# nihalsid/single-view-3d-reconstruction

Hardware: AMD Instinct MI355X
Metric: query-points/sec fwd+bwd (128^3 grid, 50k pts) (higher is better)
Workload: dtype f32

## Files before the change

include/svr_hip.h:

```cpp
#ifndef SVR_HIP_H
#define SVR_HIP_H

#include <stdint.h>

#ifdef __cplusplus
extern "C" {
#endif

#define SVR_OK 0
#define SVR_E_BADARG (-1)
#define SVR_E_BADSHAPE (-2)
#define SVR_E_ALIGN (-3)
#define SVR_E_UNSUPPORTED (-4)
#define SVR_E_IO (-5)
#define SVR_E_NOTFOUND (-6)

#define SVR_MAX_LEVELS 6

int svr_version(void);
const char *svr_last_error(void);

typedef struct svr_pull_plan {
  const uint32_t *keys;
  const void *recs;
  const int32_t *heads;
  int64_t n_items;
} svr_pull_plan;

typedef struct svr_level {
  const float *vol;
  float *gvol;
  int32_t C, D, H, W;
  int32_t col;
  const int32_t *order;
  const int32_t *item_order;
  const svr_pull_plan *plan;
} svr_level;

typedef struct svr_gather_desc {
  int32_t n_levels;
  int32_t B, N;
  int32_t row_stride;
  int32_t align_corners;
  float displacement;
  const int32_t *order;
  svr_level level[SVR_MAX_LEVELS];
  int32_t flags;
} svr_gather_desc;

#define SVR_GATHER_WIDE_OFFSETS 1
#define SVR_GATHER_DETERMINISTIC 2

int64_t svr_sizeof_level(void);
int64_t svr_sizeof_gather_desc(void);

int svr_points_voxel_order(const float *points, int32_t *order, int32_t B, int32_t N, int32_t D, int32_t H,
                           int32_t W, int32_t align_corners, void *workspace, void *stream);
int64_t svr_points_morton_order_workspace(int32_t B, int32_t N);
int svr_points_morton_order(const float *points, int32_t *order, float *sorted_points ,
                            int32_t B, int32_t N, void *workspace, void *stream);

int64_t svr_gather_pull_plan_workspace(int32_t B, int32_t N);
int64_t svr_gather_pull_plan_workspace_cells(int32_t B, int32_t D, int32_t H, int32_t W);
int svr_gather_pull_plan(const float *points, int32_t B, int32_t N, int32_t D, int32_t H, int32_t W, int32_t C,
                         int32_t col, int32_t row_stride, int32_t align_corners, float displacement,
                         uint32_t *keys, void *recs, int32_t *heads, int32_t *items , int32_t *stats ,
                         void *workspace, void *stream);

int svr_gather_item_order(const float *points, int32_t B, int32_t N, int32_t D, int32_t H, int32_t W,
                          int32_t align_corners, float displacement, int32_t with_j ,
                          int32_t *items, void *workspace, void *stream);
int svr_gather_item_order_xblock(const float *points, int32_t B, int32_t N, int32_t D, int32_t H, int32_t W,
                                 int32_t align_corners, float displacement, int32_t block, int32_t *items,
                                 void *workspace, void *stream);
int svr_gather_project_bwd(const float *points, const float *dh, int64_t lddh, int32_t B, int32_t N, int32_t D, int32_t H,
                           int32_t W, int32_t align_corners, float displacement, const int32_t *items, float *dP,
                           void *stream);

int64_t svr_gather_project_plan_workspace(int32_t B, int32_t N);
int64_t svr_gather_project_slots(int32_t B, int32_t N, int32_t D, int32_t H, int32_t W);
int svr_gather_project_plan(const float *points, int32_t B, int32_t N, int32_t D, int32_t H, int32_t W, int32_t align_corners,
                            float displacement, int32_t *items, uint32_t *keys, int32_t *sidx, int32_t *first_slot,
                            void *workspace, void *stream);
int svr_gather_project_bwd2(const float *points, const float *dh, int64_t lddh, int32_t B, int32_t N, int32_t D, int32_t H,
                            int32_t W, int32_t align_corners, float displacement, const int32_t *items, const int32_t *sidx,
                            const int32_t *first_slot, float *partials, float *dP, void *stream);

int svr_gather_trilinear_fwd(const svr_gather_desc *d, const float *points ,
                             float *features, void *stream);
int32_t svr_gather_fc0_supported(const svr_gather_desc *d);
int64_t svr_gather_fc0_workspace(const svr_gather_desc *d, int32_t n_out);
int svr_gather_fc0_fwd(const svr_gather_desc *d, const float *points, const float *W, int64_t ldw, const float *bias, float *Y,
                       int64_t ldy, int32_t n_out, float *features, int64_t ldf, const int32_t *keep_cols, uint32_t keep_levels,
                       int32_t epilogue, void *workspace, void *stream);
int svr_gather_fc0_prepare(const svr_gather_desc *d, const float *W, int64_t ldw, int32_t n_out, float *features, int64_t ldf,
                           const int32_t *keep_cols, uint32_t keep_levels, void *workspace, void *stream);
int svr_gather_fc0_run(const svr_gather_desc *d, const float *points, const float *bias, float *Y, int64_t ldy, int32_t n_out,
                       float *features, int64_t ldf, const int32_t *keep_cols, uint32_t keep_levels, int32_t epilogue,
                       void *workspace, void *stream);
int svr_gather_fc0_bf16_prepare(const svr_gather_desc *d, const float *W, int64_t ldw, int32_t n_out, void *workspace,
                                void *stream);
int svr_gather_fc0_bf16_run(const svr_gather_desc *d, const float *points, const float *bias, uint16_t *Y, int64_t ldy,
                            int32_t n_out, int32_t epilogue, void *workspace, void *stream);
int svr_gather_trilinear_bwd(const svr_gather_desc *d, const float *points, const float *gfeatures,
                             float *gpoints, void *stream);
int svr_gather_corner_indices(const svr_gather_desc *d, int32_t level, const float *points,
                              int32_t *out, void *stream);

int svr_cast_f32_to_bf16(const float *in, uint16_t *out, int64_t n, void *stream);
int svr_gather_trilinear_fwd_bf16(const svr_gather_desc *d, const float *points, uint16_t *features, void *stream);
int svr_linear_fwd_bf16(const uint16_t *X, int64_t ldx, const uint16_t *W, int64_t ldw, const float *bias, uint16_t *Y,
                        int64_t ldy, int64_t M, int64_t N, int64_t K, int epilogue, void *stream);
int svr_fc_out_fwd_bf16(const uint16_t *H, int64_t ldh, const float *w, const float *b, float *logits,
                        const int32_t *row_map, int64_t M, int64_t K, void *stream);

#define SVR_EPI_NONE 0
#define SVR_EPI_BIAS 1
#define SVR_EPI_BIAS_RELU 2
#define SVR_EPI_MASK 3

int svr_linear_fwd(const float *X, int64_t ldx, const float *W, int64_t ldw, const float *bias,
                   float *Y, int64_t ldy, int64_t M, int64_t N, int64_t K, int epilogue,
                   const float *mask, int64_t ldmask, void *stream);
int svr_linear_bwd_data(const float *dY, int64_t lddy, const float *W, int64_t ldw, float *dX,
                        int64_t lddx, int64_t M, int64_t N, int64_t K, int epilogue,
                        const float *mask, int64_t ldmask, void *stream);
int64_t svr_linear_bwd_weight_workspace(int64_t M, int64_t N, int64_t K);
int svr_linear_bwd_weight(const float *dY, int64_t lddy, const float *X, int64_t ldx, float *dW,
                          int64_t lddw, float *db, int64_t M, int64_t N, int64_t K,
                          void *workspace, void *stream);

int64_t svr_linear_fwd_bf16x6_workspace(int64_t N, int64_t K);
int svr_linear_fwd_bf16x6(const float *X, int64_t ldx, const float *W, int64_t ldw, const float *bias,
                          float *Y, int64_t ldy, int64_t M, int64_t N, int64_t K, int epilogue,
// ... 366 lines not shown
```

single-view-3d-reconstruction_amd/_lib.py:

```python
import ctypes as C
import os

import numpy as np
import torch

_HERE = os.path.dirname(os.path.abspath(__file__))
LIB_PATH = os.path.join(_HERE, "lib", "libsvr_hip.so")

SVR_MAX_LEVELS = 6
EPI_NONE, EPI_BIAS, EPI_BIAS_RELU, EPI_MASK = 0, 1, 2, 3

P = C.c_void_p
I32, I64, F32 = C.c_int32, C.c_int64, C.c_float


class Conv2dDesc(C.Structure):
    _fields_ = [("src0", P), ("src1", P), ("B", I32), ("H", I32), ("W", I32), ("C0", I32), ("C1", I32), ("k", I32),
                ("stride", I32), ("act", I32), ("upsample", I32)]


class PullPlan(C.Structure):
    _fields_ = [("keys", P), ("recs", P), ("heads", P), ("n_items", I64)]


class Level(C.Structure):
    _fields_ = [("vol", P), ("gvol", P), ("C", I32), ("D", I32), ("H", I32), ("W", I32), ("col", I32), ("order", P),
                ("item_order", P), ("plan", C.POINTER(PullPlan))]


class GatherDesc(C.Structure):
    _fields_ = [("n_levels", I32), ("B", I32), ("N", I32), ("row_stride", I32), ("align_corners", I32),
                ("displacement", F32), ("order", P), ("level", Level * SVR_MAX_LEVELS), ("flags", I32)]


GATHER_WIDE_OFFSETS, GATHER_DETERMINISTIC = 1, 2
EVAL_SUMS_WORKSPACE_BYTES = 6144


SIGNATURES = {
    "svr_version": (C.c_int, []),
    "svr_last_error": (C.c_char_p, []),
    "svr_sizeof_level": (I64, []),
    "svr_sizeof_gather_desc": (I64, []),
    "svr_points_morton_order_workspace": (I64, [I32, I32]),
    "svr_points_morton_order": (C.c_int, [P, P, P, I32, I32, P, P]),
    "svr_points_voxel_order": (C.c_int, [P, P, I32, I32, I32, I32, I32, I32, P, P]),
    "svr_gather_item_order": (C.c_int, [P, I32, I32, I32, I32, I32, I32, F32, I32, P, P, P]),
    "svr_gather_item_order_xblock": (C.c_int, [P, I32, I32, I32, I32, I32, I32, F32, I32, P, P, P]),
    "svr_gather_project_bwd": (C.c_int, [P, P, I64, I32, I32, I32, I32, I32, I32, F32, P, P, P]),
    "svr_gather_project_plan_workspace": (C.c_int64, [I32, I32]),
    "svr_gather_project_slots": (C.c_int64, [I32, I32, I32, I32, I32]),
    "svr_gather_project_plan": (C.c_int, [P, I32, I32, I32, I32, I32, I32, F32, P, P, P, P, P, P]),
    "svr_gather_project_bwd2": (C.c_int, [P, P, I64, I32, I32, I32, I32, I32, I32, F32, P, P, P, P, P, P]),
    "svr_gather_pull_plan_workspace": (I64, [I32, I32]),
    "svr_gather_pull_plan_workspace_cells": (I64, [I32, I32, I32, I32]),
    "svr_gather_pull_plan": (C.c_int, [P, I32, I32, I32, I32, I32, I32, I32, I32, I32, F32, P, P, P, P, P, P, P]),
    "svr_gather_trilinear_fwd": (C.c_int, [C.POINTER(GatherDesc), P, P, P]),
    "svr_gather_fc0_supported": (C.c_int32, [C.POINTER(GatherDesc)]),
    "svr_gather_fc0_workspace": (C.c_int64, [C.POINTER(GatherDesc), I32]),
    "svr_gather_fc0_fwd": (C.c_int, [C.POINTER(GatherDesc), P, P, I64, P, P, I64, I32, P, I64, P, C.c_uint32, I32, P, P]),
    "svr_gather_fc0_prepare": (C.c_int, [C.POINTER(GatherDesc), P, I64, I32, P, I64, P, C.c_uint32, P, P]),
    "svr_gather_fc0_run": (C.c_int, [C.POINTER(GatherDesc), P, P, P, I64, I32, P, I64, P, C.c_uint32, I32, P, P]),
    "svr_gather_fc0_bf16_prepare": (C.c_int, [C.POINTER(GatherDesc), P, I64, I32, P, P]),
    "svr_gather_fc0_bf16_run": (C.c_int, [C.POINTER(GatherDesc), P, P, P, I64, I32, I32, P, P]),
    "svr_gather_trilinear_bwd": (C.c_int, [C.POINTER(GatherDesc), P, P, P, P]),
    "svr_gather_corner_indices": (C.c_int, [C.POINTER(GatherDesc), I32, P, P, P]),
    "svr_cast_f32_to_bf16": (C.c_int, [P, P, I64, P]),
    "svr_gather_trilinear_fwd_bf16": (C.c_int, [C.POINTER(GatherDesc), P, P, P]),
    "svr_linear_fwd_bf16": (C.c_int, [P, I64, P, I64, P, P, I64, I64, I64, I64, C.c_int, P]),
    "svr_fc_out_fwd_bf16": (C.c_int, [P, I64, P, P, P, P, I64, I64, P]),
    "svr_linear_fwd": (C.c_int, [P, I64, P, I64, P, P, I64, I64, I64, I64, C.c_int, P, I64, P]),
    "svr_linear_bwd_data": (C.c_int, [P, I64, P, I64, P, I64, I64, I64, I64, C.c_int, P, I64, P]),
    "svr_linear_bwd_weight_workspace": (I64, [I64, I64, I64]),
    "svr_linear_bwd_weight": (C.c_int, [P, I64, P, I64, P, I64, P, I64, I64, I64, P, P]),
    "svr_linear_fwd_bf16x6_workspace": (I64, [I64, I64]),
    "svr_linear_fwd_bf16x6": (C.c_int, [P, I64, P, I64, P, P, I64, I64, I64, I64, C.c_int, P, P]),
    "svr_linear_fwd_f16x3_workspace": (I64, [I64, I64]),
    "svr_linear_fwd_f16x3": (C.c_int, [P, I64, P, I64, P, P, I64, I64, I64, I64, C.c_int, P, P]),
    "svr_linear_bwd_data_bf16x3_workspace": (I64, [I64, I64]),
    "svr_linear_bwd_data_bf16x3": (C.c_int, [P, I64, P, I64, P, I64, I64, I64, I64, C.c_int, P, I64, P, P]),
    "svr_linear_bwd_weight_bf16x3_workspace": (I64, [I64, I64, I64]),
    "svr_linear_bwd_weight_bf16x3": (C.c_int, [P, I64, P, I64, P, I64, P, I64, I64, I64, P, P]),
    "svr_amax_f32": (C.c_int, [P, I64, I64, I64, P, P]),
    "svr_linear_bwd_data_f16x3_workspace": (I64, [I64, I64]),
    "svr_linear_bwd_data_f16x3": (C.c_int, [P, I64, P, I64, P, I64, I64, I64, I64, C.c_int, P, I64, P, P, P, P]),
    "svr_linear_bwd_weight_f16x3_workspace": (I64, [I64, I64, I64]),
    "svr_linear_bwd_weight_f16x3": (C.c_int, [P, I64, P, I64, P, I64, P, I64, I64, I64, P, P, P]),
    "svr_linear_variant": (C.c_int, [I32, I64, I64, I64, I64, I64, I64, I64, I32, I32, I32, I32, I32, I32, P, P, P, P, P, P]),
    "svr_fc_out_fwd": (C.c_int, [P, I64, P, P, P, P, I64, I64, P]),
    "svr_fc_out_bwd_workspace": (I64, [I64, I64]),
    "svr_fc_out_bwd": (C.c_int, [P, I64, P, P, P, P, I64, P, P, I64, I64, P, P, P]),
    "svr_bce_logits_sum_mean": (C.c_int, [P, P, P, P, I64, I64, F32, P, P]),
    "svr_bce_ordered_workspace": (I64, [I64]),
    "svr_bce_logits_sum_mean_ordered": (C.c_int, [P, P, P, P, I64, I64, F32, P, P]),
    "svr_conv3d_pack_weight": (C.c_int, [P, P, P, I32, I32, P]),
    "svr_conv3d_unpack_wgrad": (C.c_int, [P, P, I32, I32, P]),
    "svr_conv3d_k3": (C.c_int, [P, P, P, P, I32, I32, I32, I32, I32, I32, C.c_int, P, P]),
    "svr_conv3d_fwd_bf16x6_workspace": (I64, [I32, I32]),
    "svr_conv3d_k3_fwd_bf16x6": (C.c_int, [P, P, P, P, I32, I32, I32, I32, I32, I32, C.c_int, P, P]),
    "svr_conv3d_fwd_f16x3_workspace": (I64, [I32, I32]),
    "svr_conv3d_k3_fwd_f16x3": (C.c_int, [P, P, P, P, I32, I32, I32, I32, I32, I32, C.c_int, P, P]),
    "svr_conv3d_fwd_f16x3_stats_blocks": (I32, [I32, I32, I32, I32, I32, I32]),
    "svr_conv3d_k3_fwd_f16x3_stats": (C.c_int, [P, P, P, P, P, I32, I32, I32, I32, I32, I32, C.c_int, P, P]),
    "svr_conv3d_bwd_data_bf16x3_workspace": (I64, [I32, I32]),
    "svr_conv3d_k3_bwd_data_bf16x3": (C.c_int, [P, P, P, I32, I32, I32, I32, I32, I32, C.c_int, P, P, P]),
    "svr_conv3d_c1_fwd_stats_workspace": (I64, [I32, I32, I32, I32, I32]),
    "svr_conv3d_c1_fwd_stats": (C.c_int, [P, P, P, P, P, I32, I32, I32, I32, I32, C.c_int, P, P]),
    "svr_conv3d_k3_bwd_weight_workspace": (I64, [I32, I32, I32, I32, I32, I32]),
    "svr_conv3d_k3_bwd_weight": (C.c_int, [P, P, P, P, I32, I32, I32, I32, I32, I32, P, P]),
    "svr_conv3d_k3_bwd_weight_bf16x3_workspace": (I64, [I32, I32, I32, I32, I32, I32]),
    "svr_conv3d_k3_bwd_weight_bf16x3": (C.c_int, [P, P, P, P, I32, I32, I32, I32, I32, I32, P, P]),
    "svr_conv3d_k3_bwd_weight_bf16x3_param": (C.c_int, [P, P, P, P, I32, I32, I32, I32, I32, I32, P, P]),
    "svr_conv3d_bwd_data_f16x3_workspace": (I64, [I32, I32]),
    "svr_conv3d_k3_bwd_data_f16x3": (C.c_int, [P, P, P, I32, I32, I32, I32, I32, I32, C.c_int, P, P, P, P, P]),
    "svr_conv3d_k3_bwd_weight_f16x3": (C.c_int, [P, P, P, P, I32, I32, I32, I32, I32, I32, I32, P, P, P]),
    "svr_conv3d_k3_variant": (C.c_int, [I32, I32, I32, I32, I32, I32, I32, P, P, P, P, P]),
    "svr_bn_stats_workspace": (I64, [I64, I32]),
    "svr_bn_stats": (C.c_int, [P, P, I64, I32, P, P]),
# ... 167 lines not shown
```

single-view-3d-reconstruction_amd/csrc/gather.hip:

```cpp
#include "common.h"
#include "gather_common.h"
#include "reduce.h"

namespace {

struct LevelArgs {
  const float *vol;
  float *gvol;
  int C, D, H, W, col;
  const int32_t *order;
  const int32_t *items;
};

struct FusedArgs {
  LevelArgs L[SVR_MAX_LEVELS];
  unsigned block_start[SVR_MAX_LEVELS + 1];
  int n;
  int pad_start;
  int shared;
  int xcd;
};

template <int C, bool JMAJOR = false>
__device__ __forceinline__ void gather_fwd_body(const LevelArgs L, const float *__restrict__ points,
// ... 715 lines not shown
}

__global__ __launch_bounds__(128) void gather_bwd_serial_kernel(LevelArgs L, const float *__restrict__ points,
                                                                const float *__restrict__ gfeat, int N,
                                                                int row_stride, float disp, int ac) {
  const int b = blockIdx.x, c = threadIdx.x;
  if (c >= L.C) return;
  float *gb = L.gvol + (size_t)b * L.D * L.H * L.W * L.C + c;
  for (int j = 0; j < 7; ++j)
    for (int n = 0; n < N; ++n) {
      const int64_t pn = (int64_t)b * N + n;
      const Corner cr = sample_corner(points + pn * 3, j, disp, L.D, L.H, L.W, ac);
      const Weights w = corner_weights(cr);
      const float g = gfeat[pn * row_stride + L.col + j * L.C + c];
#pragma unroll
      for (int k = 0; k < 8; ++k) {
        const int z = w.z0 + (k >> 2), y = w.y0 + ((k >> 1) & 1), x = w.x0 + (k & 1);
        if (z >= 0 && z < L.D && y >= 0 && y < L.H && x >= 0 && x < L.W) {
          volatile float *q = gb + (((size_t)z * L.H + y) * L.W + x) * L.C;
          *q = *q + corner_w(w, k) * g;
        }
      }
    }
}

struct PullRec {
  float fx, fy, fz;
  int32_t goff;
};

__device__ __forceinline__ bool pull_cell(const float *pt, int j, float disp, int D, int H, int W, int ac, int b,
                                          uint32_t &key, float &fx, float &fy, float &fz) {
  const Corner c = sample_corner(pt, j, disp, D, H, W, ac);
  const int x0 = clamp_int(c.x0f), y0 = clamp_int(c.y0f), z0 = clamp_int(c.z0f);
  fx = c.ix - c.x0f;
  fy = c.iy - c.y0f;
  fz = c.iz - c.z0f;
  if (!(z0 >= -1 && z0 < D && y0 >= -1 && y0 < H && x0 >= -1 && x0 < W)) return false;
  key = (uint32_t)((((int64_t)b * (D + 1) + z0 + 1) * (H + 1) + y0 + 1) * (W + 1) + x0 + 1);
  return true;
}

__global__ __launch_bounds__(256) void pull_key_kernel(const float *__restrict__ points, uint32_t *__restrict__ keys,
                                                       int32_t *__restrict__ vals, int64_t total, int N, int D, int H,
                                                       int W, float disp, int ac, uint32_t sentinel, int kblk) {
  const int64_t i = (int64_t)blockIdx.x * 256 + threadIdx.x;
  if (i >= total) return;
  const int64_t pn = i / 7;
  const int j = (int)(i - pn * 7);
  uint32_t key;
  float fx, fy, fz;
  const float p3[3] = {points[pn * 3], points[pn * 3 + 1], points[pn * 3 + 2]};
  const bool ok = pull_cell(p3, j, disp, D, H, W, ac, (int)(pn / N), key, fx, fy, fz);
  if (ok && kblk > 0) {
    const uint32_t w1 = (uint32_t)W + 1u, K = (uint32_t)kblk, row = key / w1, x = key - row * w1;
    key = ((row * ((w1 + K - 1u) / K) + x / K) * 8u + (uint32_t)j) * K + x % K;
  }
  keys[i] = ok ? key : sentinel;
  vals[i] = (int32_t)i;
}

__global__ __launch_bounds__(256) void pull_record_kernel(const float *__restrict__ points,
                                                          const uint32_t *__restrict__ keys,
                                                          const int32_t *__restrict__ items, PullRec *__restrict__ recs,
                                                          int32_t *__restrict__ ends, int64_t total, int N, int D, int H,
                                                          int W, int C, int col, int row_stride, float disp, int ac,
                                                          uint32_t sentinel) {
  const int64_t idx = (int64_t)blockIdx.x * 256 + threadIdx.x;
  if (idx >= total) return;
  const uint32_t k = keys[idx];
  if (k == sentinel) return;
  const int32_t id = items[idx];
  const int32_t pn = id / 7;
  const int j = id - pn * 7;
  const float p3[3] = {points[(int64_t)pn * 3], points[(int64_t)pn * 3 + 1], points[(int64_t)pn * 3 + 2]};
  uint32_t key;
  PullRec r;
  pull_cell(p3, j, disp, D, H, W, ac, pn / N, key, r.fx, r.fy, r.fz);
  r.goff = pn * row_stride + col + j * C;
  recs[idx] = r;
  if (idx == total - 1 || keys[idx + 1] != k) ends[k + 1] = (int32_t)idx + 1;
}

template <int C, int XS, int BZ, int BY, int BXG>
__global__ __launch_bounds__(256) void gather_bwd_pull_kernel(float *__restrict__ gvol, const uint32_t *__restrict__ keys,
                                                              const PullRec *__restrict__ recs,
                                                              const int32_t *__restrict__ cs,
                                                              const float *__restrict__ gfeat, int n_items, int B, int D,
                                                              int H, int W) {
  constexpr int V = C / 4;
  static_assert(BZ * BY * BXG * V == 256, "brick must fill the workgroup");
  const int t = threadIdx.x;
  const int q4 = (t % V) * 4, si = t / V;
  const int nbx = (W + BXG * XS - 1) / (BXG * XS), nby = (H + BY - 1) / BY, nbz = (D + BZ - 1) / BZ;
  uint32_t bid = blockIdx.x;
  const int bx = bid % nbx; bid /= nbx;
  const int by = bid % nby; bid /= nby;
  const int bz = bid % nbz;
  const int b = bid / nbz;
  const int x0 = (bx * BXG + si % BXG) * XS, y = by * BY + (si / BXG) % BY, z = bz * BZ + si / (BXG * BY);
  if (x0 >= W || y >= H || z >= D) return;
  const int ncell = min(XS, W - x0) + 1;
  uint32_t kbase[4];
  int lo[4], hi[4];
#pragma unroll
  for (int w = 0; w < 4; ++w) {
    const int dz = w >> 1, dy = w & 1;
    kbase[w] = (uint32_t)((((int64_t)b * (D + 1) + z + dz) * (H + 1) + y + dy) * (W + 1) + x0);
    lo[w] = cs[kbase[w]];
    hi[w] = cs[kbase[w] + ncell];
  }
  float4 acc[XS];
#pragma unroll
  for (int i = 0; i < XS; ++i) acc[i] = make_float4(0.f, 0.f, 0.f, 0.f);
  const int last = n_items - 1;
  while (lo[0] < hi[0] || lo[1] < hi[1] || lo[2] < hi[2] || lo[3] < hi[3]) {
    uint32_t k[4];
    PullRec r[4];
#pragma unroll
    for (int w = 0; w < 4; ++w) {
      const int i = min(lo[w], last);
      k[w] = keys[i];
      r[w] = recs[i];
    }
    float4 g[4];
    bool v[4];
#pragma unroll
    for (int w = 0; w < 4; ++w) {
      v[w] = lo[w] < hi[w];
      g[w] = *reinterpret_cast<const float4 *>(gfeat + (v[w] ? r[w].goff : 0) + q4);
    }
#pragma unroll
    for (int w = 0; w < 4; ++w) {
      const int dz = w >> 1, dy = w & 1;
      if (v[w]) {
        const int o = (int)(k[w] - kbase[w]);
        const float wyz = (dy ? 1.f - r[w].fy : r[w].fy) * (dz ? 1.f - r[w].fz : r[w].fz);
        const float wa = r[w].fx * wyz, wb = (1.f - r[w].fx) * wyz;
#pragma unroll
        for (int i = 0; i < XS; ++i) {
          const float wt = (o == i) ? wa : ((o == i + 1) ? wb : 0.f);
          acc[i].x += wt * g[w].x; acc[i].y += wt * g[w].y; acc[i].z += wt * g[w].z; acc[i].w += wt * g[w].w;
        }
        ++lo[w];
      }
    }
  }
  float *out = gvol + ((((int64_t)b * D + z) * H + y) * W + x0) * C + q4;
#pragma unroll
  for (int i = 0; i < XS; ++i)
    if (x0 + i < W) *reinterpret_cast<float4 *>(out + (int64_t)i * C) = acc[i];
}

template <int XS>
__global__ __launch_bounds__(256) void gather_bwd_pull_c1_kernel(float *__restrict__ gvol, const uint32_t *__restrict__ keys,
                                                                 const PullRec *__restrict__ recs,
                                                                 const int32_t *__restrict__ cs,
                                                                 const float *__restrict__ gfeat, int n_items,
                                                                 int64_t strips, int D, int H, int W) {
  const int64_t t = (int64_t)blockIdx.x * 256 + threadIdx.x;
  if (t >= strips) return;
  const int nsx = (W + XS - 1) / XS;
  const int x0 = (int)(t % nsx) * XS;
  int64_t q = t / nsx;
  const int y = (int)(q % H); q /= H;
  const int z = (int)(q % D);
  const int64_t b = q / D;
  const int ncell = min(XS, W - x0) + 1;
  uint32_t kbase[4];
  int lo[4], hi[4];
#pragma unroll
  for (int w = 0; w < 4; ++w) {
    const int dz = w >> 1, dy = w & 1;
    kbase[w] = (uint32_t)(((b * (D + 1) + z + dz) * (H + 1) + y + dy) * (W + 1) + x0);
    lo[w] = cs[kbase[w]];
    hi[w] = cs[kbase[w] + ncell];
  }
  float acc[XS];
#pragma unroll
  for (int i = 0; i < XS; ++i) acc[i] = 0.f;
  const int last = n_items > 0 ? n_items - 1 : 0;
  while (lo[0] < hi[0] || lo[1] < hi[1] || lo[2] < hi[2] || lo[3] < hi[3]) {
    uint32_t k[4];
    PullRec r[4];
#pragma unroll
    for (int w = 0; w < 4; ++w) {
      const int i = min(lo[w], last);
      k[w] = keys[i];
      r[w] = recs[i];
    }
    float g[4];
    bool v[4];
#pragma unroll
    for (int w = 0; w < 4; ++w) {
      v[w] = lo[w] < hi[w];
      g[w] = gfeat[v[w] ? r[w].goff : 0];
    }
#pragma unroll
    for (int w = 0; w < 4; ++w) {
      const int dz = w >> 1, dy = w & 1;
      if (v[w]) {
        const int o = (int)(k[w] - kbase[w]);
        const float wyz = (dy ? 1.f - r[w].fy : r[w].fy) * (dz ? 1.f - r[w].fz : r[w].fz);
        const float wa = r[w].fx * wyz, wb = (1.f - r[w].fx) * wyz;
#pragma unroll
        for (int i = 0; i < XS; ++i) {
          const float wt = (o == i) ? wa : ((o == i + 1) ? wb : 0.f);
          acc[i] += wt * g[w];
        }
        ++lo[w];
      }
    }
  }
  float *out = gvol + ((b * D + z) * H + y) * (int64_t)W + x0;
#pragma unroll
  for (int i = 0; i < XS; ++i)
    if (x0 + i < W) out[i] = acc[i];
}

__host__ __device__ inline int pull_xs(int C) { return C == 16 ? 8 : 4; }

__global__ __launch_bounds__(256) void pull_stats_kernel(const int32_t *__restrict__ cs, int32_t *__restrict__ stats, int B, int D,
                                                         int H, int W, int XS) {
  const int nsx = (W + XS - 1) / XS;
  const int64_t total = (int64_t)B * (D + 1) * (H + 1) * nsx, i = (int64_t)blockIdx.x * 256 + threadIdx.x;
  int len = 0;
  if (i < total) {
    const int sx = (int)(i % nsx);
    const int64_t row = i / nsx;
    const int x0 = sx * XS, ncell = min(XS, W - x0) + 1;
// ... 50 lines not shown
                                        void *stream) {
  if (int rc = check_desc(d, false)) return rc;
  if ((int64_t)d->B * d->N == 0) return SVR_OK;
  SVR_CHECK(points && features, SVR_E_BADARG, "gather_fwd: null points/features");
  SVR_CHECK(((uintptr_t)features & 15) == 0, SVR_E_ALIGN, "gather_fwd: features not 16-byte aligned");
  hipStream_t s = (hipStream_t)stream;
  int64_t BN = (int64_t)d->B * d->N;
  if (BN == 0) return SVR_OK;
  FusedArgs A;
  A.n = 0;
  unsigned blocks = 0;
  bool shared = BN * (int64_t)d->row_stride < (1LL << 31) && !(d->flags & SVR_GATHER_WIDE_OFFSETS);
  for (int l = 0; l < d->n_levels; ++l)
    if ((int64_t)d->B * d->level[l].D * d->level[l].H * d->level[l].W * d->level[l].C >= (1LL << 31)) shared = false;
  A.shared = shared ? 1 : 0;
  for (int pass = 0; pass < 2; ++pass)
    for (int l = d->n_levels - 1; l >= 0; --l) {
      if ((d->level[l].C >= 4) != (pass == 0)) continue;
      LevelArgs L = level_args(d->level[l]);
      int V = L.C >= 4 ? L.C / 4 : 1;
      A.L[A.n] = L;
      A.block_start[A.n] = blocks;
      blocks += svr::xcd_grid((shared && L.C >= 16) ? svr::cdiv(BN * 7, 256) : svr::cdiv(BN * 7 * V, 256));
      ++A.n;
    }
  A.block_start[A.n] = blocks;
  static const int xcd_order = getenv("SVR_GATHER_XCD") ? 1 : 0;
  A.xcd = xcd_order;
  A.pad_start = 0;
  for (int l = 0; l < d->n_levels; ++l) {
    int end = d->level[l].col + 7 * d->level[l].C;
    if (end > A.pad_start) A.pad_start = end;
  }
  hipLaunchKernelGGL(gather_fwd_fused_kernel, dim3(blocks), dim3(256), 0, s, A, points, features, d->order, BN, d->N,
                     d->row_stride, d->displacement, d->align_corners);
  return svr::launch_status("gather_fwd");
}

extern "C" int svr_gather_trilinear_bwd(const svr_gather_desc *d, const float *points, const float *gfeatures,
                                        float *gpoints, void *stream) {
  if (int rc = check_desc(d, true)) return rc;
  if ((int64_t)d->B * d->N == 0) return SVR_OK;
  SVR_CHECK(points && gfeatures, SVR_E_BADARG, "gather_bwd: null points/gfeatures");
  hipStream_t s = (hipStream_t)stream;
  int64_t BN = (int64_t)d->B * d->N;
  if (BN == 0) return SVR_OK;
  if (gpoints) {
    hipError_t e = hipMemsetAsync(gpoints, 0, (size_t)BN * 3 * sizeof(float), s);
    SVR_CHECK(e == hipSuccess, (int)e, "gather_bwd: memset failed: %s", hipGetErrorString(e));
  }
  FusedArgs FA;
  FA.n = 0;
  unsigned fblocks = 0;
  for (int l = d->n_levels - 1; l >= 0; --l) {
    LevelArgs L = level_args(d->level[l]);
    bool gv = L.gvol != nullptr;
    if (!gv && !gpoints) continue;
    SVR_CHECK(L.vol != nullptr || !gpoints, SVR_E_BADARG, "gather_bwd: level %d needs vol for the point gradient", l);
    if (gpoints) {
      int V = L.C >= 4 ? L.C / 4 : 1;
      int64_t total = BN * 7 * V;
      unsigned grid = (unsigned)svr::cdiv(total, 256);
      DISPATCH_C(L.C, hipLaunchKernelGGL((gather_bwd_kernel<CC, false, true>), dim3(grid), dim3(256), 0, s, L, points,
                                         gfeatures, gpoints, total, d->N, d->row_stride, d->displacement,
                                         d->align_corners));
    }
    if (!gv) continue;
    if (d->level[l].plan && !(d->flags & SVR_GATHER_DETERMINISTIC)) {
      const svr_pull_plan *P = d->level[l].plan;
      SVR_CHECK(L.C == 1 || L.C == 16 || L.C == 32 || L.C == 64, SVR_E_UNSUPPORTED, "gather_bwd: level %d: pull plan with C=%d", l,
                L.C);
      SVR_CHECK(P->keys && P->recs && P->heads && P->n_items == 7 * BN, SVR_E_BADARG, "gather_bwd: level %d: bad pull plan", l);
      SVR_CHECK(P->n_items < (1LL << 31) && BN * (int64_t)d->row_stride < (1LL << 31), SVR_E_UNSUPPORTED,
                "gather_bwd: level %d: pull plan needs 32-bit item / gradient offsets", l);
      const int n = (int)P->n_items;
      const PullRec *recs = (const PullRec *)P->recs;
#define SVR_PULL(CC, XS, BZ, BY, BXG)                                                                                     \
  {                                                                                                                       \
    const int64_t blocks = (int64_t)d->B * svr::cdiv(L.D, BZ) * svr::cdiv(L.H, BY) * svr::cdiv(L.W, BXG * XS);            \
    SVR_CHECK(blocks < (1LL << 31), SVR_E_UNSUPPORTED, "gather_bwd: level %d: %ld pull workgroups", l, (long)blocks);     \
    hipLaunchKernelGGL((gather_bwd_pull_kernel<CC, XS, BZ, BY, BXG>), dim3((unsigned)blocks), dim3(256), 0, s, L.gvol,    \
                       P->keys, recs, P->heads, gfeatures, n, d->B, L.D, L.H, L.W);                                       \
  }
      if (L.C == 1) {
        const int64_t strips = (int64_t)d->B * L.D * L.H * svr::cdiv(L.W, 4);
        SVR_CHECK(strips < (1LL << 31), SVR_E_UNSUPPORTED, "gather_bwd: level %d: %ld pull strips", l, (long)strips);
        hipLaunchKernelGGL((gather_bwd_pull_c1_kernel<4>), dim3((unsigned)svr::cdiv(strips, 256)), dim3(256), 0, s, L.gvol, P->keys,
                           recs, P->heads, gfeatures, n, strips, L.D, L.H, L.W);
      } else if (L.C == 16) SVR_PULL(16, 8, 4, 4, 4)
      else if (L.C == 32) SVR_PULL(32, 4, 2, 4, 4)
      else SVR_PULL(64, 4, 2, 2, 4)
#undef SVR_PULL
      continue;
    }
    if (d->flags & SVR_GATHER_DETERMINISTIC) {
      hipLaunchKernelGGL(gather_bwd_serial_kernel, dim3((unsigned)d->B), dim3(128), 0, s, L, points, gfeatures, d->N,
                         d->row_stride, d->displacement, d->align_corners);
      continue;
    }
    if (L.C == 1) {
      int64_t total = BN * 7;
      hipLaunchKernelGGL((gather_bwd_kernel<1, true, false>), dim3((unsigned)svr::cdiv(total, 256)), dim3(256), 0, s, L,
                         points, gfeatures, gpoints, total, d->N, d->row_stride, d->displacement, d->align_corners);
      continue;
    }
    FA.L[FA.n] = L;
    FA.block_start[FA.n] = fblocks;
    SVR_CHECK(L.D < 1022 && L.H < 1022 && L.W < 1022, SVR_E_UNSUPPORTED, "gather_bwd: level %d: dims above 1021", l);
    if (L.items) {
      SVR_CHECK(7 * BN < (1LL << 31) && BN * (int64_t)d->row_stride < (1LL << 31), SVR_E_UNSUPPORTED,
                "gather_bwd: level %d: item order needs 32-bit item / gradient offsets", l);
      fblocks += (unsigned)svr::cdiv(bwd_items_waves(L.C, 7 * BN) * 64, 256);
    } else {
      fblocks += (unsigned)svr::cdiv(bwd_runs_waves(L.C, d->B, d->N) * 64, 256);
    }
    ++FA.n;
  }
  if (FA.n > 0) {
    FA.block_start[FA.n] = fblocks;
    hipLaunchKernelGGL(gather_bwd_fused_kernel, dim3(fblocks), dim3(256), 0, s, FA, points, gfeatures, d->order, d->B, d->N,
                       d->row_stride, d->displacement, d->align_corners);
  }
  return svr::launch_status("gather_bwd");
}

extern "C" int svr_gather_corner_indices(const svr_gather_desc *d, int32_t level, const float *points,
                                         int32_t *out, void *stream) {
  if (int rc = check_desc(d, false)) return rc;
  SVR_CHECK(level >= 0 && level < d->n_levels, SVR_E_BADARG, "corner_indices: level %d", level);
  SVR_CHECK(points && out, SVR_E_BADARG, "corner_indices: null pointer");
  const svr_level &L = d->level[level];
  int64_t total = (int64_t)d->B * 7 * d->N;
  if (total == 0) return SVR_OK;
  hipLaunchKernelGGL(corner_index_kernel, dim3((unsigned)svr::cdiv(total, 256)), dim3(256), 0, (hipStream_t)stream,
                     points, out, total, d->N, L.D, L.H, L.W, d->displacement, d->align_corners);
  return svr::launch_status("corner_indices");
}

extern "C" int64_t svr_gather_pull_plan_workspace(int32_t B, int32_t N) {
  const int64_t T = (int64_t)7 * B * N;
  if (T <= 0) return 256;
  return 3 * svr::align256(T * 4) + svr::align256((int64_t)svr::sort_pairs_u32_temp_bytes(T, 32)) + 256;
}

extern "C" int64_t svr_gather_pull_plan_workspace_cells(int32_t B, int32_t D, int32_t H, int32_t W) {
  const int64_t cells = pull_cells(B, D, H, W);
  return svr::align256((cells + 1) * 4) + svr::align256((int64_t)svr::scan_max_i32_temp_bytes(cells + 1)) + 256;
}

extern "C" int svr_gather_pull_plan(const float *points, int32_t B, int32_t N, int32_t D, int32_t H, int32_t W, int32_t C,
                                    int32_t col, int32_t row_stride, int32_t align_corners, float displacement,
                                    uint32_t *keys, void *recs, int32_t *heads, int32_t *items_out, int32_t *stats,
                                    void *workspace, void *stream) {
  const int64_t T = (int64_t)7 * B * N;
  SVR_CHECK(B >= 0 && N >= 0 && D > 0 && H > 0 && W > 0, SVR_E_BADSHAPE, "pull_plan: B=%d N=%d dims %dx%dx%d", B, N, D, H, W);
  SVR_CHECK(heads && workspace, SVR_E_BADARG, "pull_plan: null heads / workspace");
  hipStream_t s = (hipStream_t)stream;
  const int64_t cells = pull_cells(B, D, H, W);
  SVR_CHECK(cells < (1LL << 31) - 1 && T < (1LL << 31) && (int64_t)B * N * row_stride < (1LL << 31), SVR_E_UNSUPPORTED,
            "pull_plan: %ld cells / %ld items / %ld gradient floats exceed 32-bit offsets", (long)cells, (long)T,
            (long)((int64_t)B * N * row_stride));
  char *w = svr::align256(workspace);
  int32_t *ends = (int32_t *)w;
  w += svr::align256((cells + 1) * 4);
  void *scan_tmp = (void *)w;
  const size_t scan_bytes = svr::scan_max_i32_temp_bytes(cells + 1);
  w += svr::align256((int64_t)scan_bytes);
  hipError_t e = hipMemsetAsync(ends, 0, (size_t)(cells + 1) * sizeof(int32_t), s);
  SVR_CHECK(e == hipSuccess, (int)e, "pull_plan: memset failed: %s", hipGetErrorString(e));
  if (T > 0) {
    SVR_CHECK(points && keys && recs, SVR_E_BADARG, "pull_plan: null pointer");
    uint32_t *keys_in = (uint32_t *)w;
    w += svr::align256(T * 4);
    int32_t *vals_in = (int32_t *)w;
    w += svr::align256(T * 4);
// ... 150 lines not shown
```

Measured before the change: 26.63 million.

## Stage pull-plan records and gradients in LDS for C=16/32 backward bricks

Adds an LDS-staged variant of the backward pull kernel for C=16 and C=32 levels. Each workgroup loads the cell heads for its brick, compacts the brick's pull records (keys and weights) into shared memory, and for C=16 also prefetches the gradient rows into LDS. The per-voxel walk then reads from LDS using a packed-index round-robin over the four neighbour rows. If a brick holds more items than the capacity, or a new flag requests it, the kernel falls back to walking global memory. The aim is to cut repeated global loads of records and gradients that neighbouring voxels share, at the cost of extra syncs, LDS pressure and lower occupancy.

```diff
diff --git a/include/svr_hip.h b/include/svr_hip.h
--- a/include/svr_hip.h
+++ b/include/svr_hip.h
@@ -50,6 +50,7 @@
 
 #define SVR_GATHER_WIDE_OFFSETS 1
 #define SVR_GATHER_DETERMINISTIC 2
+#define SVR_GATHER_PULL_GLOBAL_WALK 4
 
 int64_t svr_sizeof_level(void);
 int64_t svr_sizeof_gather_desc(void);
diff --git a/single-view-3d-reconstruction_amd/_lib.py b/single-view-3d-reconstruction_amd/_lib.py
--- a/single-view-3d-reconstruction_amd/_lib.py
+++ b/single-view-3d-reconstruction_amd/_lib.py
@@ -33,7 +33,7 @@
                 ("displacement", F32), ("order", P), ("level", Level * SVR_MAX_LEVELS), ("flags", I32)]
 
 
-GATHER_WIDE_OFFSETS, GATHER_DETERMINISTIC = 1, 2
+GATHER_WIDE_OFFSETS, GATHER_DETERMINISTIC, GATHER_PULL_GLOBAL_WALK = 1, 2, 4
 EVAL_SUMS_WORKSPACE_BYTES = 6144
 
 
diff --git a/single-view-3d-reconstruction_amd/csrc/gather.hip b/single-view-3d-reconstruction_amd/csrc/gather.hip
--- a/single-view-3d-reconstruction_amd/csrc/gather.hip
+++ b/single-view-3d-reconstruction_amd/csrc/gather.hip
@@ -821,6 +821,93 @@
   if (idx == total - 1 || keys[idx + 1] != k) ends[k + 1] = (int32_t)idx + 1;
 }
 
+struct PullFromGlobal {
+  const uint32_t *keys;
+  const PullRec *recs;
+  const float *gfeat;
+  int q4;
+  __device__ __forceinline__ void item(int i, uint32_t &k, PullRec &r) const { k = keys[i]; r = recs[i]; }
+  __device__ __forceinline__ float4 grad(int, const PullRec &r, bool valid) const {
+    return *reinterpret_cast<const float4 *>(gfeat + (valid ? r.goff : 0) + q4);
+  }
+};
+struct PullRecsFromLds {
+  const uint32_t *keys;
+  const float4 *recs;
+  const float *gfeat;
+  int q4;
+  __device__ __forceinline__ void item(int i, uint32_t &k, PullRec &r) const {
+    const float4 f = recs[i];
+    k = keys[i];
+    r = PullRec{f.x, f.y, f.z, __float_as_int(f.w)};
+  }
+  __device__ __forceinline__ float4 grad(int, const PullRec &r, bool valid) const {
+    return *reinterpret_cast<const float4 *>(gfeat + (valid ? r.goff : 0) + q4);
+  }
+};
+
+template <int XS, class Src>
+__device__ __forceinline__ void pull_walk(float4 (&acc)[XS], int (&lo)[4], const int (&hi)[4], const uint32_t (&kbase)[4],
+                                          int last, const Src src) {
+  while (lo[0] < hi[0] || lo[1] < hi[1] || lo[2] < hi[2] || lo[3] < hi[3]) {
+    uint32_t k[4];
+    PullRec r[4];
+    int idx[4];
+#pragma unroll
+    for (int w = 0; w < 4; ++w) {
+      idx[w] = min(lo[w], last);
+      src.item(idx[w], k[w], r[w]);
+    }
+    float4 g[4];
+    bool v[4];
+#pragma unroll
+    for (int w = 0; w < 4; ++w) {
+      v[w] = lo[w] < hi[w];
+      g[w] = src.grad(idx[w], r[w], v[w]);
+    }
+#pragma unroll
+    for (int w = 0; w < 4; ++w) {
+      const int dz = w >> 1, dy = w & 1;
+      if (v[w]) {
+        const int o = (int)(k[w] - kbase[w]);
+        const float wyz = (dy ? 1.f - r[w].fy : r[w].fy) * (dz ? 1.f - r[w].fz : r[w].fz);
+        const float wa = r[w].fx * wyz, wb = (1.f - r[w].fx) * wyz;
+#pragma unroll
+        for (int i = 0; i < XS; ++i) {
+          const float wt = (o == i) ? wa : ((o == i + 1) ? wb : 0.f);
+          acc[i].x += wt * g[w].x; acc[i].y += wt * g[w].y; acc[i].z += wt * g[w].z; acc[i].w += wt * g[w].w;
+        }
+        ++lo[w];
+      }
+    }
+  }
+}
+
+template <int XS, int STRIDE4>
+__device__ __forceinline__ void pull_walk_lds(float4 (&acc)[XS], const int (&lo)[4], const int (&hi)[4], int c0,
+                                              const uint32_t *cx, const float4 *recs, const float4 *g4) {
+  uint32_t cur = (uint32_t)lo[0] | (uint32_t)lo[1] << 8 | (uint32_t)lo[2] << 16 | (uint32_t)lo[3] << 24;
+  const uint32_t end = (uint32_t)hi[0] | (uint32_t)hi[1] << 8 | (uint32_t)hi[2] << 16 | (uint32_t)hi[3] << 24;
+  uint32_t open = (lo[0] < hi[0] ? 1u : 0u) | (lo[1] < hi[1] ? 2u : 0u) | (lo[2] < hi[2] ? 4u : 0u) | (lo[3] < hi[3] ? 8u : 0u);
+  uint32_t w = 3;
+  while (open) {
+    w = (w + 1 + __builtin_ctz((open | open << 4) >> (w + 1))) & 3;
+    const uint32_t sh = w * 8, i = (cur >> sh) & 0xFFu;
+    cur += 1u << sh;
+    if (i + 1 == ((end >> sh) & 0xFFu)) open &= ~(1u << w);
+    const float4 r = recs[i];
+    const float4 g = g4[i * STRIDE4];
+    const int o = (int)cx[i] - c0;
+    const float wyz = ((w & 1) ? 1.f - r.y : r.y) * ((w & 2) ? 1.f - r.z : r.z);
+    const float wa = r.x * wyz, wb = (1.f - r.x) * wyz;
+#pragma unroll
+    for (int v = 0; v < XS; ++v) {
+      const float wt = (o == v) ? wa : ((o == v + 1) ? wb : 0.f);
+      acc[v].x += wt * g.x; acc[v].y += wt * g.y; acc[v].z += wt * g.z; acc[v].w += wt * g.w;
+    }
+  }
+}
+
 template <int C, int XS, int BZ, int BY, int BXG>
 __global__ __launch_bounds__(256) void gather_bwd_pull_kernel(float *__restrict__ gvol, const uint32_t *__restrict__ keys,
                                                               const PullRec *__restrict__ recs,
@@ -885,6 +972,101 @@
       }
     }
   }
+  float *out = gvol + ((((int64_t)b * D + z) * H + y) * W + x0) * C + q4;
+#pragma unroll
+  for (int i = 0; i < XS; ++i)
+    if (x0 + i < W) *reinterpret_cast<float4 *>(out + (int64_t)i * C) = acc[i];
+}
+
+template <int C, int XS, int BZ, int BY, int BXG, int CAP, bool GRADS>
+__global__ __launch_bounds__(256) void gather_bwd_pull_lds_kernel(float *__restrict__ gvol, const uint32_t *__restrict__ keys,
+                                                                  const PullRec *__restrict__ recs,
+                                                                  const int32_t *__restrict__ cs,
+                                                                  const float *__restrict__ gfeat, int n_items, int B, int D,
+                                                                  int H, int W, int global_walk) {
+  constexpr int V = C / 4, ROWS = (BZ + 1) * (BY + 1), HS = BXG * XS + 2, GS = C + 4;
+  constexpr int LPR = ROWS <= 16 ? 16 : (ROWS <= 32 ? 8 : 4);
+  static_assert(BZ * BY * BXG * V == 256, "brick must fill the workgroup");
+  static_assert(ROWS * LPR <= 256 && ROWS + 1 <= 256, "one lane group per cell row");
+  static_assert(!GRADS || CAP <= 255, "pull_walk_lds packs four local indices into a register");
+  __shared__ int32_t s_head[ROWS * HS];
+  __shared__ int32_t s_off[ROWS + 1];
+  __shared__ uint32_t s_key[CAP];
+  __shared__ float4 s_rec[CAP];
+  __shared__ float4 s_g[GRADS ? CAP * GS / 4 : 1];
+  static_assert(sizeof(s_head) + sizeof(s_off) + sizeof(s_key) + sizeof(s_rec) + sizeof(s_g) <= 64 * 1024, "LDS budget");
+  const int t = threadIdx.x;
+  const int q4 = (t % V) * 4, si = t / V;
+  const int nbx = (W + BXG * XS - 1) / (BXG * XS), nby = (H + BY - 1) / BY, nbz = (D + BZ - 1) / BZ;
+  uint32_t bid = blockIdx.x;
+  const int bx = bid % nbx; bid /= nbx;
+  const int by = bid % nby; bid /= nby;
+  const int bz = bid % nbz;
+  const int b = bid / nbz;
+  const int xb = bx * BXG * XS, yb = by * BY, zb = bz * BZ;
+  const int ncx = min(BXG * XS, W - xb) + 1;
+  for (int e = t; e < ROWS * HS; e += 256) {
+    const int r = e / HS, c = min(e - r * HS, ncx);
+    const int cz = zb + r / (BY + 1), cy = yb + r % (BY + 1);
+    s_head[e] = (cz <= D && cy <= H) ? cs[(((int64_t)b * (D + 1) + cz) * (H + 1) + cy) * (W + 1) + xb + c] : 0;
+  }
+  __syncthreads();
+  if (t <= ROWS) {
+    int off = 0;
+    for (int r = 0; r < t; ++r) off += s_head[r * HS + HS - 1] - s_head[r * HS];
+    s_off[t] = off;
+  }
+  __syncthreads();
+  const int n = s_off[ROWS];
+  const bool staged = n <= CAP && !global_walk;
+  if (staged) {
+    if (t < ROWS * LPR) {
+      const int r = t / LPR, src = s_head[r * HS], dst = s_off[r], len = s_off[r + 1] - dst;
+      const uint32_t krow = (uint32_t)((((int64_t)b * (D + 1) + zb + r / (BY + 1)) * (H + 1) + yb + r % (BY + 1)) * (W + 1) + xb);
+      for (int j = t % LPR; j < len; j += LPR) {
+        const PullRec rec = recs[src + j];
+        s_key[dst + j] = keys[src + j] - krow;
+        s_rec[dst + j] = make_float4(rec.fx, rec.fy, rec.fz, __int_as_float(rec.goff));
+      }
+    }
+    __syncthreads();
+    if (GRADS && n > 0) {
+      constexpr int PASSES = (CAP * V + 255) / 256;
+      float4 g[PASSES];
+#pragma unroll
+      for (int p = 0; p < PASSES; ++p) {
+        const int it = min((p * 256 + t) / V, n - 1);
+        g[p] = *reinterpret_cast<const float4 *>(gfeat + __float_as_int(s_rec[it].w) + q4);
+      }
+#pragma unroll
+      for (int p = 0; p < PASSES; ++p) {
+        const int it = (p * 256 + t) / V;
+        if (it < n) s_g[it * (GS / 4) + t % V] = g[p];
+      }
+      __syncthreads();
+    }
+  }
+  const int x0 = xb + (si % BXG) * XS, y = yb + (si / BXG) % BY, z = zb + si / (BXG * BY);
+  if (x0 >= W || y >= H || z >= D) return;
+  const int ncell = min(XS, W - x0) + 1;
+  uint32_t kbase[4];
+  int lo[4], hi[4];
+#pragma unroll
+  for (int w = 0; w < 4; ++w) {
+    const int dz = w >> 1, dy = w & 1;
+    const int r = (z - zb + dz) * (BY + 1) + (y - yb + dy), h = r * HS + (x0 - xb);
+    kbase[w] = staged ? (uint32_t)(x0 - xb)
+                      : (uint32_t)((((int64_t)b * (D + 1) + z + dz) * (H + 1) + y + dy) * (W + 1) + x0);
+    const int local = staged ? s_off[r] - s_head[r * HS] : 0;
+    lo[w] = s_head[h] + local;
+    hi[w] = s_head[h + ncell] + local;
+  }
+  float4 acc[XS];
+#pragma unroll
+  for (int i = 0; i < XS; ++i) acc[i] = make_float4(0.f, 0.f, 0.f, 0.f);
+  if (!staged) pull_walk<XS>(acc, lo, hi, kbase, n_items - 1, PullFromGlobal{keys, recs, gfeat, q4});
+  else if (GRADS) pull_walk_lds<XS, GS / 4>(acc, lo, hi, x0 - xb, s_key, s_rec, s_g + t % V);
+  else pull_walk<XS>(acc, lo, hi, kbase, max(n - 1, 0), PullRecsFromLds{s_key, s_rec, gfeat, q4});
   float *out = gvol + ((((int64_t)b * D + z) * H + y) * W + x0) * C + q4;
 #pragma unroll
   for (int i = 0; i < XS; ++i)
@@ -1101,15 +1283,24 @@
     hipLaunchKernelGGL((gather_bwd_pull_kernel<CC, XS, BZ, BY, BXG>), dim3((unsigned)blocks), dim3(256), 0, s, L.gvol,    \
                        P->keys, recs, P->heads, gfeatures, n, d->B, L.D, L.H, L.W);                                       \
   }
+#define SVR_PULL_LDS(CC, XS, BZ, BY, BXG, CAP, GRADS)                                                                     \
+  {                                                                                                                       \
+    const int64_t blocks = (int64_t)d->B * svr::cdiv(L.D, BZ) * svr::cdiv(L.H, BY) * svr::cdiv(L.W, BXG * XS);            \
+    SVR_CHECK(blocks < (1LL << 31), SVR_E_UNSUPPORTED, "gather_bwd: level %d: %ld pull workgroups", l, (long)blocks);     \
+    hipLaunchKernelGGL((gather_bwd_pull_lds_kernel<CC, XS, BZ, BY, BXG, CAP, GRADS>), dim3((unsigned)blocks), dim3(256),  \
+                       0, s, L.gvol, P->keys, recs, P->heads, gfeatures, n, d->B, L.D, L.H, L.W,                          \
+                       (d->flags & SVR_GATHER_PULL_GLOBAL_WALK) ? 1 : 0);                                                 \
+  }
       if (L.C == 1) {
         const int64_t strips = (int64_t)d->B * L.D * L.H * svr::cdiv(L.W, 4);
         SVR_CHECK(strips < (1LL << 31), SVR_E_UNSUPPORTED, "gather_bwd: level %d: %ld pull strips", l, (long)strips);
         hipLaunchKernelGGL((gather_bwd_pull_c1_kernel<4>), dim3((unsigned)svr::cdiv(strips, 256)), dim3(256), 0, s, L.gvol, P->keys,
                            recs, P->heads, gfeatures, n, strips, L.D, L.H, L.W);
-      } else if (L.C == 16) SVR_PULL(16, 8, 4, 4, 4)
-      else if (L.C == 32) SVR_PULL(32, 4, 2, 4, 4)
+      } else if (L.C == 16) SVR_PULL_LDS(16, 8, 4, 4, 4, 255, true)
+      else if (L.C == 32) SVR_PULL_LDS(32, 4, 2, 4, 4, 512, false)
       else SVR_PULL(64, 4, 2, 2, 4)
 #undef SVR_PULL
+#undef SVR_PULL_LDS
       continue;
     }
     if (d->flags & SVR_GATHER_DETERMINISTIC) {
```

New measurement: 26.66 million, median of 6. No clear change (+0.1%).
